# saforem2/l2hmc

Hardware: AMD Instinct MI355X
Metric: leapfrog-steps/sec (whole node), 8x8 U(1) batch 2048, 10 LF (higher is better)
Workload: dtype f32; 1 GPU; U(1) 8x8 lattice, beta=2.0, batch 2048 per GPU, 10 LF steps, GenericNet H=512 (BASELINE.json configs[2]); global_batch=2048, num_steps=10, parallelism=chains sharded over 1 GPU(s) (weak scaling), weights replicated

## Files before the change

include/l2hmc_hip.h:

```cpp
#ifndef L2HMC_HIP_H
#define L2HMC_HIP_H

#include <stddef.h>
#include <stdint.h>

#ifdef __cplusplus
extern "C" {
#endif

#define L2HMC_OK 0
#define L2HMC_ERR_ARG 1
#define L2HMC_ERR_HIP 2
#define L2HMC_ERR_WORKSPACE 3

#define L2HMC_ABI_VERSION 1

typedef void* l2hmc_stream_t;

int l2hmc_abi_version(void);
const char* l2hmc_last_error(void);

int l2hmc_u1_action_force(const float* x, int64_t rows, int32_t T, int32_t X, float beta,
                          float* action, float* force, float* avg_plaq, float* top_charge,
                          l2hmc_stream_t stream);
// ... 49 lines not shown
int l2hmc_lf_update_v(const float* v, const float* grad, const float* S, const float* T,
                      const float* Q, float eps, int32_t dir, int64_t rows, int32_t D,
                      float* v_out, float* logdet, l2hmc_stream_t stream);
int l2hmc_lf_update_x(const float* x, const float* v, const float* keep, const float* S,
                      const float* T, const float* Q, float eps, int32_t dir, int64_t rows,
                      int32_t D, float* x_out, float* logdet, l2hmc_stream_t stream);

int l2hmc_accept_prob(const float* h_old, const float* h_new, const float* sumlogdet, int64_t n,
                      float* p, l2hmc_stream_t stream);

int l2hmc_mix_accept(const float* x, const float* xf, const float* vf, const float* pf,
                     const float* xb, const float* vb, const float* pb, const float* coin,
                     const float* u, int32_t strict, int64_t B, int32_t D, float* x_prop,
                     float* v_prop, float* p, float* x_out, l2hmc_stream_t stream);

#define L2HMC_PLAN_LAYERED 1
#define L2HMC_PLAN_CONV3D 2
#define L2HMC_PLAN_SELECTED_ONLY 4
#define L2HMC_PLAN_RECOMPUTE 8
#define L2HMC_PLAN_TILES16_ONLY 16
#define L2HMC_PLAN_ALL_COLUMNS 32
#define L2HMC_PLAN_FULL_L1 64
#define L2HMC_PLAN_SINGLE_KICKS 128
typedef struct l2hmc_gauge_plan {
  int32_t T, X;
  int32_t num_steps;
  int32_t hmc;
  float eps;
  int32_t flags;
  const float* masks;
  l2hmc_dense_net xnet;
  l2hmc_dense_net vnet;
  l2hmc_conv3d_front xfront;
  l2hmc_conv3d_front vfront;
  const void* heads;
} l2hmc_gauge_plan;

size_t l2hmc_gauge_pack_heads_bytes(const l2hmc_gauge_plan* plan);
int l2hmc_gauge_pack_heads(const l2hmc_gauge_plan* plan, void* heads, l2hmc_stream_t stream);

size_t l2hmc_gauge_ws_bytes(const l2hmc_gauge_plan* plan, int64_t rows);

int l2hmc_gauge_plan_fused(const l2hmc_gauge_plan* plan);

int l2hmc_gauge_step_plan(int64_t rows_all, int32_t cus, int64_t* rows_out, int32_t* rows_per_wg_out);

// ... 207 lines not shown
```

l2hmc_amd/_lib.py:

```python
import ctypes as C
import os
import re

import torch

_HERE = os.path.dirname(os.path.abspath(__file__))
LIB_PATH = os.environ.get("L2HMC_LIB_PATH") or os.path.join(_HERE, "libl2hmc_hip.so")
HEADER_PATH = os.path.join(os.path.dirname(_HERE), "include", "l2hmc_hip.h")

c_float_p = C.c_void_p
MAX_MIX, MAX_SMALL_DIM, MAX_SMALL_NODES = 8, 8, 64
PLAN_LAYERED, PLAN_CONV3D, PLAN_SELECTED_ONLY, PLAN_RECOMPUTE, PLAN_TILES16_ONLY, PLAN_ALL_COLUMNS = 1, 2, 4, 8, 16, 32
PLAN_FULL_L1 = 64
PLAN_SINGLE_KICKS = 128
GRAD_BUCKET_REST = 6
BUCKET_FN = C.CFUNCTYPE(None, C.c_void_p, C.c_int32)


class DenseNet(C.Structure):
    _fields_ = [("D", C.c_int32), ("H", C.c_int32), ("Ka", C.c_int32), ("Kb", C.c_int32),
                ("w1_t", c_float_p), ("wt", c_float_p), ("b1", c_float_p), ("wh_t", c_float_p),
                ("bh", c_float_p), ("whd_t", c_float_p), ("bhd", c_float_p),
                ("coeff_s", c_float_p), ("coeff_q", c_float_p),
                ("q_tanh", C.c_int32), ("reserved", C.c_int32), ("packed", c_float_p)]


class DenseGrads(C.Structure):
    _fields_ = [(n, c_float_p) for n in ("w1_t", "wt", "b1", "wh_t", "bh", "whd_t", "bhd", "coeff_s", "coeff_q")]


class Conv3DGrads(C.Structure):
    _fields_ = [(n, c_float_p) for n in ("w1_a", "b1_a", "w2_a", "b2_a", "w1_b", "b1_b", "w2_b", "b2_b")]


class Conv3DFront(C.Structure):
    _fields_ = [("F", C.c_int32), ("reserved", C.c_int32),
                ("w1_a", c_float_p), ("b1_a", c_float_p), ("w2_a", c_float_p), ("b2_a", c_float_p),
# ... 228 lines not shown
```

l2hmc_amd/csrc/fused_args.h:

```cpp
#pragma once
#include "stq_dense.h"

namespace l2hmc {

struct FusedArgs {
  int T, X, num_steps, step_begin, step_end;
  float eps, beta;
  const float* masks;
  l2hmc_dense_net xnet, vnet;
  l2hmc_conv3d_front xfront, vfront;
  const float* x0; const float* v0;
  const int* dir;
  int64_t x_mod;
  int64_t dir_split;
  int64_t rows;
  float* x_out; float* v_out;
  float* logdet;
  int logdet_accumulate;
  float* p_accept;
  unsigned long long* stamps;
  int stagger;
  FusedTape tx, tv;
  float* step_x_next;
  float* step_xprop; float* step_vprop; float* step_xout;
  int64_t step_B;
  int64_t step_Bl, step_chain0;
  int step_sums_acc;
  unsigned long long step_seed, step_draw;
  int step_both;
  float* step_px; float* step_act; float* step_plq; float* step_chg; float* step_dq;
  float* step_sums;
  float* step_part;
  int step_split;
  float* step_hand;
  int* step_ticket;
  const int* heads_meta;
  const float* heads_img;
  const float* l1_img;
  int single_kicks;
};

size_t fused4_pack_floats(const l2hmc_dense_net* n);
int launch_fused4_pack(const l2hmc_dense_net* n, float* image4, hipStream_t stream);
int fused4_rows_per_wg(int64_t rows, int cus);
int launch_fused4(const FusedArgs& a, int rows_per_wg, hipStream_t stream);

int fused32_supported(const l2hmc_dense_net* n);
int launch_fused32(const FusedArgs& a, hipStream_t stream);

}
```

l2hmc_amd/csrc/fused_common.h:

```cpp
#pragma once
#include "stq_dense.h"
#include <math.h>

namespace l2hmc {

using f32x4 = __attribute__((ext_vector_type(4))) float;

constexpr int kFM = 16;
#ifndef L2HMC_FUSED_WAVES
#define L2HMC_FUSED_WAVES 4
#endif
constexpr int kFWaves = L2HMC_FUSED_WAVES;
constexpr int kFThreads = 64 * kFWaves;
constexpr int kTPC = kFThreads / kFM;


#ifdef L2HMC_TAPE_TEMPORAL
__device__ __forceinline__ void tape_store(float* dst, const f32x4& v) { *reinterpret_cast<f32x4*>(dst) = v; }
__device__ __forceinline__ f32x4 tape_load(const float* src) { return *reinterpret_cast<const f32x4*>(src); }
#else
__device__ __forceinline__ void tape_store(float* dst, const f32x4& v) {
  __builtin_nontemporal_store(v, reinterpret_cast<f32x4*>(dst));
}
__device__ __forceinline__ f32x4 tape_load(const float* src) {
// ... 32 lines not shown

template <int NT, int DEPTH, int NTI = NT, int TS = 1>
__device__ __forceinline__ void ring_prime(BRing<NT, DEPTH>& R, const float* __restrict__ wp, bool rev = false,
                                           int nkc = 0, int toff = 0) {
  const WSection ws = wsection(wp);
#pragma unroll
  for (int s = 0; s < DEPTH - 1; ++s) load_frags<NT, NTI, TS>(R.b[s], ws, rev ? nkc - 1 - s : s, toff);
  load_group<NT, 0, (NT + 1) / 2, NTI, TS>(R.b[DEPTH - 1], ws, rev ? nkc - DEPTH : DEPTH - 1, toff);
}

template <int G, int NLD, int MPL = 4, int g = 0>
__device__ __forceinline__ void sched_mfma_load_pipeline() {
  if constexpr (g < G) {
    __builtin_amdgcn_sched_group_barrier(0x008, MPL, 0);
    if constexpr (g < NLD) __builtin_amdgcn_sched_group_barrier(0x020, g == G - 1 ? NLD - g : 1, 0);
    sched_mfma_load_pipeline<G, NLD, MPL, g + 1>();
  }
}

template <int NT, int T0, int T1, int L0, int L1, bool LOAD, int NDS = 0, int NTI = NT, int TS = 1>
__device__ __forceinline__ void mfma_half_stream(const f32x4 a, const f32x4 (&cur)[NT], f32x4 (&dst)[NT],
                                                 f32x4 (&acc)[NT], const WSection& wp, int kc, int toff = 0) {
  constexpr int G = T1 - T0, NLD = L1 - L0;
#pragma unroll
  for (int i = 0; i < 4 * G; ++i) {
    const int e = i / G, t = T0 + i % G;
    acc[t] = __builtin_amdgcn_mfma_f32_16x16x4f32(cur[t][e], a[e], acc[t], 0, 0, 0);
  }
  if constexpr (LOAD) {
#pragma unroll
    for (int j = 0; j < NLD; ++j) dst[L0 + j] = lane_frag(wp, (unsigned)(kc * NTI + toff + (L0 + j) * TS));
  }
  if constexpr (NDS > 0) __builtin_amdgcn_sched_group_barrier(0x100, NDS, 0);
  sched_mfma_load_pipeline<G, LOAD ? NLD : 0>();
}

template <int NT, int NKC, int DEPTH, int NTI = NT, int TS = 1, typename AF>
__device__ __forceinline__ void stream_layer(BRing<NT, DEPTH>& R, const float* __restrict__ wbase, AF afrag,
                                             f32x4 (&acc)[NT], bool rev = false, int toff = 0) {
  const WSection wp = wsection(wbase);
  static_assert(DEPTH >= 2 && NKC >= DEPTH && NT >= 2, "ring depth / tile groups");
  constexpr int G = (NT + 1) / 2;
  auto km = [&](int k) { return rev ? NKC - 1 - k : k; };
  constexpr int MAIN = (NKC - DEPTH) / DEPTH * DEPTH;
  __builtin_amdgcn_sched_barrier(0);
  f32x4 a0 = afrag(km(0));
  int kc = 0;
#pragma nounroll
  for (; kc < MAIN; kc += DEPTH) {
#pragma unroll
    for (int s = 0; s < DEPTH; ++s) {
      const f32x4 a1 = afrag(km(kc + s + 1));
      mfma_half_stream<NT, 0, G, G, NT, true, 1, NTI, TS>(a0, R.b[s], R.b[(s + DEPTH - 1) % DEPTH], acc, wp,
                                                          km(kc + s + DEPTH - 1), toff);
      mfma_half_stream<NT, G, NT, 0, G, true, 0, NTI, TS>(a0, R.b[s], R.b[s], acc, wp, km(kc + s + DEPTH), toff);
      a0 = a1;
    }
  }
#pragma unroll
  for (int k = MAIN; k < NKC; ++k) {
    const int s = (k - MAIN) % DEPTH;
    const f32x4 a1 = afrag(km(k + 1 < NKC ? k + 1 : NKC - 1));
    if (k + DEPTH - 1 < NKC)
      mfma_half_stream<NT, 0, G, G, NT, true, 1, NTI, TS>(a0, R.b[s], R.b[(s + DEPTH - 1) % DEPTH], acc, wp,
// ... 14 lines not shown
```

l2hmc_amd/csrc/fused_traj.hip:

```cpp
#include "fused_step.h"
#include "lf_update.h"
#include <atomic>
#include <stdlib.h>

namespace l2hmc {

template <int D, int H, int KA = D, bool CONV = false>
struct FusedCfg {
  static constexpr int IMGW = CONV ? 2 * kFWaves : kFWaves;
  static constexpr int WAVES = 2 * kFWaves;
  static constexpr int RW = WAVES / IMGW;
  static constexpr int THREADS = 64 * WAVES;
  static constexpr int TPC = CONV ? THREADS / kFM : 16;
  static constexpr int SX = D + 8;
  static constexpr int SA = KA + 8;
  static constexpr int SH = H + 8;
  static constexpr int NT1 = H / (16 * WAVES);
  static constexpr int NTH = D / (16 * WAVES);
  static constexpr int NTI1 = H / (16 * IMGW);
  static constexpr int NTIH = D / (16 * IMGW);
  static_assert(NT1 >= 1 && NT1 <= 8 && NTH >= 1, "every wave needs at least one tile per layer");
  static_assert(RW == 1 || NTH == 1, "a shared heads section is walked with one tile per head and wave");
  static constexpr int KC1 = 2 * KA / 16;
  static constexpr int KC2 = H / 16;
  static constexpr size_t P1 = (size_t)2 * KA * H;
  static constexpr size_t P2 = (size_t)H * H;
  static constexpr size_t PH = (size_t)3 * D * H;
  static constexpr int NC = 4 * H + 5 * D;
  static constexpr int CF = 8, CL = 8;
  static constexpr int CW = 18 * CF + CF + 8 * CF * CF + 2 * CF;
  static constexpr int CXIN = (CL + 2) * (CL + 2) * 2;
  static constexpr int CP1 = (CL / 2 + 1) * (CL / 2 + 1) * CF;
  static constexpr int CONV_FLOATS = CONV ? 2 * kFM * SA + 4 * CW + kFM * (CXIN + CP1) : 0;
  static constexpr int ACT_FLOATS = CONV ? 0 : kFM * SX + D + 4 + D + 2 * kFM;
  static constexpr int LDS_FLOATS = 3 * kFM * SX + 2 * kFM * SH + 2 * NC + kFM * (D / 2 + 4)  +
                                    2 * D  + WAVES * kFM  + (RW > 1 ? IMGW * 64 : 0)  + kFM  +
                                    8 * kFM  + CONV_FLOATS + ACT_FLOATS;
};

__global__ void pack_fused_kernel(l2hmc_dense_net n, float* __restrict__ out, int waves) {
  const int kFWaves = waves;
  const int D = n.D, H = n.H, K1 = n.Ka + n.Kb;
  const size_t P1 = (size_t)K1 * H, P2 = (size_t)H * H, PH = (size_t)3 * D * H;
  const int NT1 = H / (16 * kFWaves), NTH = D / (16 * kFWaves);
  for (size_t i = (size_t)blockIdx.x * blockDim.x + threadIdx.x; i < P1 + P2 + PH;
       i += (size_t)gridDim.x * blockDim.x) {
    const int j = (int)(i & 3), lane = (int)((i >> 2) & 63);
    size_t rest;
    float val;
    if (i < P1 + P2) {
      const bool first = i < P1;
      const int K = first ? K1 : H;
      rest = (first ? i : i - P1) >> 8;
      const int t = (int)(rest % NT1);
      rest /= NT1;
      const int KC = K / 16;
      const int kc = (int)(rest % KC), w = (int)(rest / KC);
      const int col = (w * NT1 + t) * 16 + (lane & 15);
      const int k = kc * 16 + (lane >> 4) * 4 + j;
      val = first ? n.w1_t[(size_t)col * K1 + k] : n.wh_t[(size_t)col * H + k];
// ... 150 lines not shown
  const int sdw = wg.sdw;
  float* spx = wg.spx;
  stage_chains<kFM, kFThreads, D, SX>(p, wg, xs, vs, sdir);
  load_consts<kFThreads, D, H>(p.xnet, cx, tid);
  load_consts<kFThreads, D, H>(p.vnet, cv, tid);
  if constexpr (CONV) {
    constexpr int F = Cfg::CF, F2 = 2 * Cfg::CF;
    auto load_filters = [&](const float* w1, const float* b1, const float* w2, const float* b2, float* dst) {
      for (int i = tid; i < 18 * F; i += kFThreads) dst[i] = w1[i];
      for (int i = tid; i < F; i += kFThreads) dst[18 * F + i] = b1[i];
      for (int i = tid; i < 4 * F * F2; i += kFThreads) {
        const int g = i % F2, c = (i / F2) % F, tap = i / (F2 * F);
        dst[19 * F + i] = w2[((size_t)(tap * 2) * F + c) * F2 + g];
      }
      for (int i = tid; i < F2; i += kFThreads) dst[19 * F + 4 * F * F2 + i] = b2[i];
    };
    load_filters(p.xfront.w1_a, p.xfront.b1_a, p.xfront.w2_a, p.xfront.b2_a, cwl + 0 * Cfg::CW);
    load_filters(p.xfront.w1_b, p.xfront.b1_b, p.xfront.w2_b, p.xfront.b2_b, cwl + 1 * Cfg::CW);
    load_filters(p.vfront.w1_a, p.vfront.b1_a, p.vfront.w2_a, p.vfront.b2_a, cwl + 2 * Cfg::CW);
    load_filters(p.vfront.w1_b, p.vfront.b1_b, p.vfront.w2_b, p.vfront.b2_b, cwl + 3 * Cfg::CW);
    for (int i = tid; i < kFM * (Cfg::CXIN + Cfg::CP1); i += kFThreads) cxin[i] = 0.f;
  }
  if (tid < IMGW * kFM) ldw[tid] = 0.f;
  if constexpr (!CONV) {
    if (tid < 2 * kFM) spz[tid] = 0.f;
  }
  __syncthreads();

  const int dirl = sdir[r];

  const ChainLanes cl = chain_lanes<kFM, kTPC, 1>(p, tid);
  float act0[1], kin0[1];
  force_pass<kFM, kTPC, 1, D, SX, SP>(cl, xs, sp, gs, act0);
  kinetic_pass<kFM, kTPC, 1, D, SX>(cl, vs, kin0);

  [[maybe_unused]] auto conv_features = [&](const float* src, const float* cw, float* dst) {
    constexpr int F = Cfg::CF, F2 = 2 * Cfg::CF, L = Cfg::CL, LP = L + 2, L2 = L / 2, L2P = L2 + 1, L4 = L / 4;
    const float* w1 = cw;
    const float* b1 = cw + 18 * F;
    const float* w2 = b1 + F;
    const float* b2 = w2 + 4 * F * F2;
    for (int i = tid; i < kFM * D; i += kFThreads) {
      const int c = i / D, e = i - c * D;
      const int site = e >> 1, mu = e & 1, ii = site / L, jj = site - ii * L;
      cxin[c * Cfg::CXIN + ((ii + 1) * LP + jj + 1) * 2 + mu] = src[c * SX + e];
    }
// ... 81 lines not shown
                  }
              }
        }
        const float m0 = fmaxf(fmaxf(acc[0][0][0], acc[0][1][0]), fmaxf(acc[1][0][0], acc[1][1][0]));
        const float m1 = fmaxf(fmaxf(acc[0][0][1], acc[0][1][1]), fmaxf(acc[1][0][1], acc[1][1][1]));
        *reinterpret_cast<f32x2*>(dst + c * SA + (I2 * L4 + J2) * F2 + 2 * gp) = f32x2{fmaxf(m0, 0.f), fmaxf(m1, 0.f)};
      }
    }
    __syncthreads();
  };

  constexpr bool KEEP1 = !CONV && !TAPE && Cfg::NTH == 1 && RW == 2 && kFWaves == 8;
  f32x4 keep_v[NT1];
  [[maybe_unused]] f32x4 keep_x_own[KEEP1 ? 1 : NT1];
  f32x4 (&keep_x)[NT1] = *[&]() {
    if constexpr (KEEP1) return &keep_v;
    else return &keep_x_own;
  }();
  bool keep_v_valid = false;
  constexpr bool ACTOK = !CONV && !TAPE && Cfg::NTH == 1 && RW == 2 && kFWaves == 8;
  int arow = 0;
  constexpr bool PAIROK = !CONV && !TAPE && Cfg::NTH == 1 && RW == 2 && kFWaves == 8;

  auto net_update = [&](const l2hmc_dense_net& net, const float* cn, const float* in1, int mode, int sub,
                        bool prep_next_mask, int l1, bool is_vnet, const float tcr, const float tsr,
                        int callidx, bool pair, const float tcr2, const float tsr2) {
    const float* pk = net.packed;
    const bool zig = (callidx & 1) != 0;
    [[maybe_unused]] const FusedTape& tp = is_vnet ? p.tv : p.tx;
    [[maybe_unused]] const size_t tcr0 = (size_t)callidx * (size_t)p.rows + (size_t)row0;
    if constexpr (TAPE) {
      {
        const float* stsrc = mode == 1 ? vs : xs;
        for (int i = tid; i < kFM * (D / 4); i += kFThreads) {
          const int rr = i / (D / 4), c4 = (i - rr * (D / 4)) * 4;
          if (rr < nrow) {
            float* dst = tp.in + (tcr0 + rr) * (2 * D);
            tape_store(dst + c4, *reinterpret_cast<const f32x4*>(in1 + rr * SX + c4));
            tape_store(dst + D + c4, *reinterpret_cast<const f32x4*>(gs + rr * SX + c4));
            tape_store(tp.st + (tcr0 + rr) * D + c4, *reinterpret_cast<const f32x4*>(stsrc + rr * SX + c4));
          }
        }
      }
    }
    [[maybe_unused]] auto tape_rows = [&](float* dst, const float* src) {
      for (int i = tid; i < kFM * (H / 4); i += kFThreads) {
// ... 5 lines not shown
    const int wv = __builtin_amdgcn_readfirstlane(wave);
    const int wimg = wv / RW, wsub = wv - wimg * RW;
    const float* wp1 = pk + (size_t)wimg * Cfg::KC1 * NTI1 * 256;
    const float* wp2 = pk + Cfg::P1 + (size_t)wimg * Cfg::KC2 * NTI1 * 256;
    const float* wph = pk + Cfg::P1 + Cfg::P2 + (size_t)wimg * Cfg::KC2 * 3 * NTIH * 256;
    const int to1 = wsub * NT1, toh = wsub * NTH;
    int asense = 0;
    bool actv = false;
    const float* wpa = nullptr;
    if (ACTOK && SPLIT && mode == 2 && p.heads_img) {
      asense = sdw ^ sub;
      actv = __builtin_amdgcn_readfirstlane(sel[asense]) != 0;
      wpa = p.heads_img + ((size_t)(arow * 2 + asense) * 4 + (wv & 3)) * Cfg::KC2 * 3 * 256;
    }
    const bool l1c = ACTOK && SPLIT && p.l1_img && p.heads_img && __builtin_amdgcn_readfirstlane(sel[0] & sel[1]) != 0;
    [[maybe_unused]] float ld_k[4] = {0.f, 0.f, 0.f, 0.f}, ld_s[4] = {0.f, 0.f, 0.f, 0.f};
#ifndef L2HMC_DP1
#define L2HMC_DP1 3
#define L2HMC_DP2 3
#define L2HMC_DPH 4
#endif
    constexpr int DP1 = L2HMC_DP1, DP2 = L2HMC_DP2, DPH = L2HMC_DPH;
    BRing<NT1, DP2> R2;
    BRing<3 * NTH, DPH> R3;
#ifndef L2HMC_DP2P
#define L2HMC_DP2P 2
#define L2HMC_DPHP 3
#endif
    constexpr int DP2P = L2HMC_DP2P, DPHP = L2HMC_DPHP;
    [[maybe_unused]] BRing<NTI1, DP2P> R2P;
    [[maybe_unused]] BRing<3 * NTIH, DPHP> R3P;
    {
      constexpr int KH = Cfg::KC1 / 2;
      f32x4 acc[NT1];
      [[maybe_unused]] unsigned long long t0 = L2HMC_CYCLES_NOW();
      const float* src1 = in1;
      const float* src2 = gs;
      int s1 = SX;
      if constexpr (CONV) {
        const float* cwn = cwl + (is_vnet ? 2 : 0) * Cfg::CW;
        [[maybe_unused]] const unsigned long long tc0 = L2HMC_CYCLES_NOW();
        if (l1 == 0 || l1 == 1 || l1 == 3) conv_features(in1, cwn, fa);
        if (l1 != 2) conv_features(gs, cwn + Cfg::CW, fb);
        L2HMC_CYCLES_ADD(ft, 8, tc0);
        src1 = fa;
        src2 = fb;
        s1 = SA;
// ... 185 lines not shown
              const f32x4 mf = *reinterpret_cast<const f32x4*>(skm + c0);
              const f32x4 mb = *reinterpret_cast<const f32x4*>(skm + D + c0);
              const f32x4 x = *reinterpret_cast<const f32x4*>(xs + idx);
              f32x4 kx;
#pragma unroll
              for (int e = 0; e < 4; ++e) kx[e] = keep_of(mf[e], mb[e], d, 0) * x[e];
              if (l1n) {
#pragma unroll
                for (int e = 0; e < 4; ++e) {
                  if (keep_of(mf[e], mb[e], d, 0) != 0.f) stg[r * SX + scp[c0 + e]] = kx[e];
                  else if (kx[e] != kx[e]) spz[r] = kx[e];
                }
              } else {
                *reinterpret_cast<f32x4*>(gs + idx) = kx;
              }
            }
          }
          L2HMC_CYCLES_ADD(ft, 5, t0);
          {
            [[maybe_unused]] const unsigned long long tb = L2HMC_CYCLES_NOW();
            __syncthreads();
            L2HMC_CYCLES_ADD(ft, 6, tb);
          }
          return;
        }
      }
      ring_prime<NT1, DP2, NTI1>(R2, wp2, zig, Cfg::KC2, to1);
      L2HMC_CYCLES_ADD(ft, 0, t0);
      t0 = L2HMC_CYCLES_NOW();
      [[maybe_unused]] unsigned gmask = 0;
#pragma unroll
      for (int t = 0; t < NT1; ++t) {
        const int c0 = (wave * NT1 + t) * 16 + q * 4;
        const f32x4 b = *reinterpret_cast<const f32x4*>(cn + c0);
        const f32x4 w0 = *reinterpret_cast<const f32x4*>(cn + H + c0);
        const f32x4 w1 = *reinterpret_cast<const f32x4*>(cn + 2 * H + c0);
        f32x4 hv;
#pragma unroll
        for (int e = 0; e < 4; ++e) {
          hv[e] = fmaxf(acc[t][e] + b[e] + (tcr * w0[e] + tsr * w1[e]), 0.f);
          if constexpr (TAPE) gmask |= (hv[e] > 0.f ? 1u : 0u) << (t * 4 + e);
        }
        *reinterpret_cast<f32x4*>(h1 + r * SH + c0) = hv;
      }
      if constexpr (TAPE) {
        const size_t word = ((size_t)(callidx * 2 + 0) * gridDim.x + blockIdx.x) * (64 * IMGW) + wimg * 64 + lane;
        if constexpr (RW == 1) tp.gate[word] = gmask;
        else reinterpret_cast<unsigned short*>(tp.gate)[word * 2 + wsub] = (unsigned short)gmask;
      }
      L2HMC_CYCLES_ADD(ft, 3, t0);
    }
    {
      [[maybe_unused]] const unsigned long long tb = L2HMC_CYCLES_NOW();
      __syncthreads();
      L2HMC_CYCLES_ADD(ft, 6, tb);
    }
    if constexpr (TAPE) tape_rows(tp.h1, h1);
    {
      f32x4 acc[NT1];
#pragma unroll
      for (int t = 0; t < NT1; ++t) acc[t] = f32x4{0.f, 0.f, 0.f, 0.f};
      const float* a = h1 + r * SH + q * 4;
      [[maybe_unused]] unsigned long long t0 = L2HMC_CYCLES_NOW();
      stream_layer<NT1, Cfg::KC2, DP2, NTI1>(
          R2, wp2, [&](int kc) { return *reinterpret_cast<const f32x4*>(a + kc * 16); }, acc, zig, to1);
      if (ACTOK && actv) {
        if (wv < 4) ring_prime<3 * NTH, DPH, 3, 1>(R3, wpa, zig, Cfg::KC2, 0);
      } else {
        ring_prime<3 * NTH, DPH, 3 * NTIH, TSH>(R3, wph, zig, Cfg::KC2, toh);
      }
      L2HMC_CYCLES_ADD(ft, 1, t0);
      t0 = L2HMC_CYCLES_NOW();
      [[maybe_unused]] unsigned gmask = 0;
#pragma unroll
      for (int t = 0; t < NT1; ++t) {
        const int c0 = (wave * NT1 + t) * 16 + q * 4;
        const f32x4 b = *reinterpret_cast<const f32x4*>(cn + 3 * H + c0);
        f32x4 hv;
#pragma unroll
        for (int e = 0; e < 4; ++e) {
          hv[e] = fmaxf(acc[t][e] + b[e], 0.f);
          if constexpr (TAPE) gmask |= (hv[e] > 0.f ? 1u : 0u) << (t * 4 + e);
        }
        *reinterpret_cast<f32x4*>(h2 + r * SH + c0) = hv;
      }
      if constexpr (TAPE) {
        const size_t word = ((size_t)(callidx * 2 + 1) * gridDim.x + blockIdx.x) * (64 * IMGW) + wimg * 64 + lane;
        if constexpr (RW == 1) tp.gate[word] = gmask;
        else reinterpret_cast<unsigned short*>(tp.gate)[word * 2 + wsub] = (unsigned short)gmask;
      }
      L2HMC_CYCLES_ADD(ft, 4, t0);
    }
    {
      [[maybe_unused]] const unsigned long long tb = L2HMC_CYCLES_NOW();
      __syncthreads();
      L2HMC_CYCLES_ADD(ft, 6, tb);
    }
    if constexpr (TAPE) tape_rows(tp.h2, h2);
    {
      f32x4 acc[3 * NTH];
#pragma unroll
      for (int t = 0; t < 3 * NTH; ++t) acc[t] = f32x4{0.f, 0.f, 0.f, 0.f};
      const float* a = h2 + r * SH + q * 4;
      [[maybe_unused]] unsigned long long t0 = L2HMC_CYCLES_NOW();
      if (ACTOK && actv) {
        if (wv < 4)
          stream_layer<3 * NTH, Cfg::KC2, DPH, 3, 1>(
              R3, wpa, [&](int kc) { return *reinterpret_cast<const f32x4*>(a + kc * 16); }, acc, zig, 0);
      } else {
        stream_layer<3 * NTH, Cfg::KC2, DPH, 3 * NTIH, TSH>(
            R3, wph, [&](int kc) { return *reinterpret_cast<const f32x4*>(a + kc * 16); }, acc, zig, toh);
      }
      L2HMC_CYCLES_ADD(ft, 2, t0);
      t0 = L2HMC_CYCLES_NOW();
      float ld = 0.f;
      const float* bhd = cn + 4 * H;
      const float* es = bhd + 3 * D;
      const float* eq = es + D;
      const int d = dirl;
      if (ACTOK && actv) {
        const int* al = scol + asense * (D / 2);
        const int* il = scol + (asense ^ 1) * (D / 2);
        if (wv < 4) {
#pragma unroll
          for (int e = 0; e < 4; ++e) {
            const int c = al[wv * 16 + q * 4 + e];
            const int idx = r * SX + c;
            float S, Tt, Q, s, omk;
            heads_stq(acc[0][e], acc[1][e], acc[2][e], bhd[c], bhd[D + c], bhd[2 * D + c], es[c], eq[c], net.q_tanh, S,
                      Tt, Q);
            const float xn = lf_drift<ExpFast>(xs[idx], vs[idx], keep_of(skm[c], skm[D + c], d, sub), S, Tt, Q, eps, d, s,
                                               omk);
            xs[idx] = xn;
            stg[idx] = omk * s;
            if (prep_next_mask) gs[l1c ? r * SX + scp[c] : idx] = omk * xn;
          }
        } else {
#pragma unroll
          for (int e = 0; e < 4; ++e) {
            const int c = il[(wv - 4) * 16 + q * 4 + e];
            const int idx = r * SX + c;
            stg[idx] = 0.f;
            if (prep_next_mask) {
              const float kx = (1.f - keep_of(skm[c], skm[D + c], d, sub)) * xs[idx];
              if (!l1c) gs[idx] = kx;
              else if (kx != kx) spz[kFM + r] = kx;
            }
          }
          if (l1c && wv == 4 && q == 0) spz[sub * kFM + r] = 0.f;
        }
      } else {
#pragma unroll
      for (int t = 0; t < NTH; ++t) {
        const int c0 = wave * (D / kFWaves) + t * 16 + q * 4;
        const f32x4 b_s = *reinterpret_cast<const f32x4*>(bhd + c0);
        const f32x4 b_t = *reinterpret_cast<const f32x4*>(bhd + D + c0);
        const f32x4 b_q = *reinterpret_cast<const f32x4*>(bhd + 2 * D + c0);
        const f32x4 e_s = *reinterpret_cast<const f32x4*>(es + c0);
        const f32x4 e_q = *reinterpret_cast<const f32x4*>(eq + c0);
        const f32x4 mf = *reinterpret_cast<const f32x4*>(skm + c0);
        const f32x4 mb = *reinterpret_cast<const f32x4*>(skm + D + c0);
        const int idx = r * SX + c0;
        f32x4 S, Tt, Q;
#pragma unroll
        for (int e = 0; e < 4; ++e) {
          float s_, t_, q_;
          heads_stq(acc[0 * NTH + t][e], acc[1 * NTH + t][e], acc[2 * NTH + t][e], b_s[e], b_t[e], b_q[e], e_s[e], e_q[e],
                    net.q_tanh, s_, t_, q_);
          S[e] = s_; Tt[e] = t_; Q[e] = q_;
        }
        if constexpr (TAPE) {
          if (r < nrow) {
            const size_t plane = (size_t)p.rows * D;
// ... 62 lines not shown
      L2HMC_CYCLES_ADD(ft, 6, tb);
    }
    if (ACTOK && actv) {
      if (wsub == 1) {
        float ld = 0.f;
#pragma unroll
        for (int h = 0; h < 2; ++h)
#pragma unroll
          for (int e = 0; e < 4; ++e) ld += stg[r * SX + (2 * wimg + h) * 16 + q * 4 + e];
        ld += __shfl_xor(ld, 16, 64);
        ld += __shfl_xor(ld, 32, 64);
        if (q == 0) ldw[wimg * kFM + r] += ld;
      }
    } else if constexpr (RW > 1) {
      if (wsub == 1) {
        float ld = ldx[wimg * 64 + lane];
#pragma unroll
        for (int e = 0; e < 4; ++e) ld += ld_k[e] * ld_s[e];
        ld += __shfl_xor(ld, 16, 64);
        ld += __shfl_xor(ld, 32, 64);
        if (q == 0) ldw[wimg * kFM + r] += ld;
      }
    }
  };

  const float two_pi = 6.28318530717958647692f;
  auto step_time = [&](int step, float& tc, float& ts) {
    const int sf = step, sb = p.num_steps - 1 - step;
    const float af = two_pi * (float)sf / (float)p.num_steps, ab = two_pi * (float)sb / (float)p.num_steps;
    const float tcf = cosf(af), tsf = sinf(af), tcb = cosf(ab), tsb = sinf(ab);
    tc = dirl ? tcb : tcf;
    ts = dirl ? tsb : tsf;
  };
  auto load_step_masks = [&](int step) {
    const int sf = step, sb = p.num_steps - 1 - step;
    for (int i = tid; i < D; i += kFThreads) {
      skm[i] = p.masks[(size_t)sf * D + i];
      skm[D + i] = p.masks[(size_t)sb * D + i];
    }
    if (ACTOK && SPLIT && p.heads_meta) {
      arow = sdw ? sb : sf;
      for (int i = tid; i < D; i += kFThreads) scol[i] = p.heads_meta[2 * p.num_steps + arow * D + i];
      if (tid < 2) sel[tid] = p.heads_meta[arow * 2 + tid];
      if (p.l1_img)
        for (int i = tid; i < D; i += kFThreads) scp[i] = p.heads_meta[2 * p.num_steps + (p.num_steps + arow) * D + i];
    }
// ... 9 lines not shown
      __syncthreads();
    }
#pragma nounroll
    for (int call = paired_in ? 1 : 0; call < 4; ++call) {
      const bool is_v = call == 0 || call == 3;
      const bool pair = pair_out && call == 3;
      if (call == 3) {
        [[maybe_unused]] const unsigned long long tf = L2HMC_CYCLES_NOW();
        float unused[1];
        force_pass<kFM, kTPC, 1, D, SX, SP>(cl, xs, sp, gs, unused);
        L2HMC_CYCLES_ADD(ft, 7, tf);
        if (pair) {
          load_step_masks(step + 1);
          step_time(step + 1, tcr2, tsr2);
        }
      }
      const int l1 = call == 0 ? (keep_v_valid ? 2 : 0) : call == 1 ? 3 : call == 2 ? 4 : 1;
      net_update(is_v ? p.vnet : p.xnet, is_v ? cv : cx, is_v ? xs : vs, is_v ? 1 : 2, call == 2 ? 1 : 0,
                 call < 2, l1, is_v, tcr, tsr, 2 * step + (call == 0 || call == 1 ? 0 : 1), pair, tcr2, tsr2);
    }
    keep_v_valid = true;
    paired_in = pair_out;
  }

  float act1[1], kin1[1];
  force_pass<kFM, kTPC, 1, D, SX, SP>(cl, xs, sp, gs, act1);
  kinetic_pass<kFM, kTPC, 1, D, SX>(cl, vs, kin1);
  if (STEPM) {
    step_accept_probs<kFM, 1, IMGW>(cl, ldw, act0, act1, kin0, kin1, spx);
    __syncthreads();
    const float* xfr = xs;
    const float* xbr = xs + (kFM / 2) * SX;
    const float* vfr = vs;
    const float* vbr = vs + (kFM / 2) * SX;
    const float* pfr = spx;
    const float* pbr = spx + kFM / 2;
    if (SPLIT) {
      constexpr int HW = 2 * kFM * D + kFM;
      float* mine = p.step_hand + (size_t)blockIdx.x * HW;
      for (int i = tid; i < kFM * (D / 4); i += kFThreads) {
        const int rr = i / (D / 4), c4 = (i - rr * (D / 4)) * 4;
        *reinterpret_cast<f32x4*>(mine + rr * D + c4) = *reinterpret_cast<const f32x4*>(xs + rr * SX + c4);
        if (p.step_vprop)
          *reinterpret_cast<f32x4*>(mine + (kFM + rr) * D + c4) = *reinterpret_cast<const f32x4*>(vs + rr * SX + c4);
      }
      if (tid < kFM) mine[2 * kFM * D + tid] = spx[tid];
// ... 235 lines not shown
  L2HMC_REQUIRE(x_in && (x_next || x_out) && B > 0 && (!step_sums || part) && hand, "fused step: bad arguments");
  const int ndir = both ? 2 : 1;
  StepPart parts[3];
  const int nparts = plan_step_parts(B * ndir, !conv && subtile_enabled(p), device_cu_count(), parts);
  auto part_of = [&](int64_t c0, int64_t nb, int rpw, int accumulate) {
    const int cpw = both ? rpw / 2 : rpw;
    const int64_t D = 2 * (int64_t)p->T * p->X;
    FusedArgs a{};
    a.T = p->T; a.X = p->X; a.num_steps = p->num_steps; a.step_begin = 0; a.step_end = p->num_steps;
    a.eps = p->eps; a.beta = beta; a.masks = p->masks; a.xnet = p->xnet; a.vnet = p->vnet;
    a.xfront = p->xfront; a.vfront = p->vfront;
    a.x0 = x_in + c0 * D; a.rows = ceil_div(nb, cpw) * rpw;
    a.step_x_next = x_next ? x_next + c0 * D : nullptr;
    a.step_xprop = x_prop ? x_prop + c0 * D : nullptr;
    a.step_vprop = v_prop ? v_prop + c0 * D : nullptr;
    a.step_xout = x_out ? x_out + c0 * D : nullptr;
    a.step_B = B; a.step_Bl = nb; a.step_chain0 = c0; a.step_sums_acc = accumulate;
    a.step_seed = seed; a.step_draw = draw; a.step_both = both;
    a.step_px = px ? px + c0 : nullptr; a.step_act = actions ? actions + c0 : nullptr;
    a.step_plq = plaqs ? plaqs + c0 : nullptr; a.step_chg = charges ? charges + c0 : nullptr;
    a.step_dq = dq ? dq + c0 : nullptr;
    a.step_sums = step_sums; a.step_part = part;
    a.single_kicks = (p->flags & L2HMC_PLAN_SINGLE_KICKS) != 0;
#ifdef L2HMC_STAMPS
    a.stamps = g_stamp_cls == 5 ? g_stamp_buf : nullptr;
    a.stagger = g_fused_stagger;
#endif
    return a;
  };
  const bool split = !conv && both;
  const int* hmeta = nullptr;
  const float* himg = nullptr;
  const float* l1img = nullptr;
  if (split && p->heads && !(p->flags & L2HMC_PLAN_ALL_COLUMNS)) {
    const int Dp = 2 * p->T * p->X;
    hmeta = reinterpret_cast<const int*>(p->heads);
    himg = reinterpret_cast<const float*>(reinterpret_cast<const char*>(p->heads) + heads_meta_bytes(p->num_steps, Dp));
    if (!(p->flags & L2HMC_PLAN_FULL_L1))
      l1img = reinterpret_cast<const float*>(reinterpret_cast<const char*>(himg) +
                                             heads_sections_bytes(p->num_steps, Dp, p->xnet.H));
  }
  auto launch16 = [&](FusedArgs a) {
    if (split) {
      const int64_t pairs = ceil_div(a.step_Bl, (int64_t)kFM);
      a.rows = 2 * pairs * kFM;
      a.step_split = 1;
// ... 80 lines not shown
```

l2hmc_amd/gauge_dynamics.py:

```python
import ctypes as C

import numpy as np
import numpy.random as npr
import torch

from . import _lib, ops
from . import autograd as _autograd
from .network import ConvNet3D, GenericNet


class GaugeDynamics:

    def __init__(self, lattice, potential_fn, **kwargs):
        self.name = 'GaugeDynamics'
        self.lattice = lattice
        self.potential = potential_fn
        self.batch_size = self.lattice.samples.shape[0]
        self.x_dim = self.lattice.num_links
        self.hmc, self.network_arch, self.num_steps = False, 'generic', 5
        self.eps_trainable, self.data_format = True, 'channels_last'
        self.both_directions = True
        self.fused = True
        self.check_numerics = False
        self.recompute = False
        self.tiles16_only = False
        self.all_columns = False
        self.full_l1 = False
        self.single_kicks = False
        for key, val in kwargs.items():
            if key != 'eps':
                setattr(self, key, val)
        self._device = kwargs.get('device') or torch.device("cuda", torch.cuda.current_device())
        if getattr(potential_fn, "u1_lattice", None) is None:
            raise NotImplementedError(
                "the fused trajectory integrates the 2D U(1) action; pass lattice.get_energy_function()")
        self.eps = torch.tensor(float(kwargs.get('eps', 0.4)), dtype=torch.float32)
        self._construct_time()
        self._construct_masks_while()
        if self.hmc:
            self.position_fn = lambda inp: [torch.zeros_like(inp[0]) for _ in range(3)]
            self.momentum_fn = lambda inp: [torch.zeros_like(inp[0]) for _ in range(3)]
        elif self.network_arch == 'generic':
            self._build_generic_nets()
        elif self.network_arch == 'conv3D':
            self._build_conv_nets_3D()
        elif self.network_arch == 'conv2D':
            raise NotImplementedError(
                "network_arch='conv2D' is out of scope (SURVEY.md section 2: not named by any benchmark "
                "config, and its 4-D outputs break the reference's own reduce_sum(axis=1))")
        else:
            raise AttributeError("`self._network_arch` must be one of `'conv3D', 'conv2D', 'generic'.`")
# ... 50 lines not shown
    @property
    def variables(self):
        v = [self.eps]
        if not self.hmc:
            v += self.position_fn.variables + self.momentum_fn.variables
        return v

    @property
    def trainable_variables(self):
        v = [self.eps] if self.eps_trainable else []
        if not self.hmc:
            v += self.position_fn.trainable_variables + self.momentum_fn.trainable_variables
        return v

    def _plan(self):
        p = _lib.GaugePlan(T=self.lattice.time_size, X=self.lattice.space_size, num_steps=self.num_steps,
                           hmc=int(bool(self.hmc)), eps=float(self.eps.detach()),
                           flags=(0 if self.fused else _lib.PLAN_LAYERED)
                           | (0 if self.both_directions else _lib.PLAN_SELECTED_ONLY)
                           | (_lib.PLAN_RECOMPUTE if self.recompute else 0)
                           | (_lib.PLAN_TILES16_ONLY if self.tiles16_only else 0)
                           | (_lib.PLAN_ALL_COLUMNS if self.all_columns else 0)
                           | (_lib.PLAN_FULL_L1 if self.full_l1 else 0)
                           | (_lib.PLAN_SINGLE_KICKS if self.single_kicks else 0),
                           masks=_lib.dev_ptr(self.mask, name="mask"))
        if not self.hmc:
            p.xnet = self.position_fn.pack()
            p.vnet = self.momentum_fn.pack()
            if self.network_arch == 'conv3D':
                p.flags |= _lib.PLAN_CONV3D
                p.xfront = self.position_fn.pack_front()
                p.vfront = self.momentum_fn.pack_front()
            elif self.fused:
                p.heads = self._heads_image(p)
        return p

    def _heads_image(self, plan):
        L = _lib.lib()
        nbytes = L.l2hmc_gauge_pack_heads_bytes(C.byref(plan))
        if not nbytes:
            return None
        key = (plan.xnet.whd_t, getattr(self.position_fn, "_pack_serial", 0))
        h = getattr(self, "_heads", None)
        if h is None or h[0] is not self.mask or h[1] != key or h[2].numel() * 4 < nbytes:
            buf = torch.empty(nbytes // 4, dtype=torch.float32, device=self._device)
            _lib.call("l2hmc_gauge_pack_heads", C.byref(plan), buf, device=self._device)
            self._heads = h = (self.mask, key, buf)
# ... 144 lines not shown
```

Before: 16.18 million chain-leapfrog-steps/s.

## Split fused head GEMM across all eight waves with LDS exchange

In the fused trajectory kernel's active-column head path, the three head output tiles were computed by waves 0-3 alone while waves 4-7 only handled the kept columns. Now waves 0-3 stream two head tiles and waves 4-7 stream the third. Partial results are swapped through LDS behind an added barrier, and every wave finishes two moved and two kept columns. This spreads head MFMA and weight streaming over twice the waves, at the cost of an extra __syncthreads and LDS traffic. The old single-wave-group behaviour is kept behind a new HEADS_ONE_WAVE plan flag, and optional per-phase stamp accumulation in LDS is added for profiling builds.

Measured after the change: 16.28 million chain-leapfrog-steps/s (median of 6 runs). No clear change (+0.6%).

```diff
diff --git a/include/l2hmc_hip.h b/include/l2hmc_hip.h
--- a/include/l2hmc_hip.h
+++ b/include/l2hmc_hip.h
@@ -95,6 +95,7 @@
 #define L2HMC_PLAN_ALL_COLUMNS 32
 #define L2HMC_PLAN_FULL_L1 64
 #define L2HMC_PLAN_SINGLE_KICKS 128
+#define L2HMC_PLAN_HEADS_ONE_WAVE 256
 typedef struct l2hmc_gauge_plan {
   int32_t T, X;
   int32_t num_steps;
diff --git a/l2hmc_amd/_lib.py b/l2hmc_amd/_lib.py
--- a/l2hmc_amd/_lib.py
+++ b/l2hmc_amd/_lib.py
@@ -13,6 +13,7 @@
 PLAN_LAYERED, PLAN_CONV3D, PLAN_SELECTED_ONLY, PLAN_RECOMPUTE, PLAN_TILES16_ONLY, PLAN_ALL_COLUMNS = 1, 2, 4, 8, 16, 32
 PLAN_FULL_L1 = 64
 PLAN_SINGLE_KICKS = 128
+PLAN_HEADS_ONE_WAVE = 256
 GRAD_BUCKET_REST = 6
 BUCKET_FN = C.CFUNCTYPE(None, C.c_void_p, C.c_int32)
 
diff --git a/l2hmc_amd/csrc/fused_args.h b/l2hmc_amd/csrc/fused_args.h
--- a/l2hmc_amd/csrc/fused_args.h
+++ b/l2hmc_amd/csrc/fused_args.h
@@ -38,6 +38,7 @@
   const float* heads_img;
   const float* l1_img;
   int single_kicks;
+  int heads_one_wave;
 };
 
 size_t fused4_pack_floats(const l2hmc_dense_net* n);
diff --git a/l2hmc_amd/csrc/fused_common.h b/l2hmc_amd/csrc/fused_common.h
--- a/l2hmc_amd/csrc/fused_common.h
+++ b/l2hmc_amd/csrc/fused_common.h
@@ -78,9 +78,10 @@
 __device__ __forceinline__ void mfma_half_stream(const f32x4 a, const f32x4 (&cur)[NT], f32x4 (&dst)[NT],
                                                  f32x4 (&acc)[NT], const WSection& wp, int kc, int toff = 0) {
   constexpr int G = T1 - T0, NLD = L1 - L0;
+  constexpr int GD = G > 0 ? G : 1;
 #pragma unroll
   for (int i = 0; i < 4 * G; ++i) {
-    const int e = i / G, t = T0 + i % G;
+    const int e = i / GD, t = T0 + i % GD;
     acc[t] = __builtin_amdgcn_mfma_f32_16x16x4f32(cur[t][e], a[e], acc[t], 0, 0, 0);
   }
   if constexpr (LOAD) {
@@ -89,13 +90,14 @@
   }
   if constexpr (NDS > 0) __builtin_amdgcn_sched_group_barrier(0x100, NDS, 0);
   sched_mfma_load_pipeline<G, LOAD ? NLD : 0>();
+  if constexpr (G == 0 && LOAD && NLD > 0) __builtin_amdgcn_sched_group_barrier(0x020, NLD, 0);
 }
 
 template <int NT, int NKC, int DEPTH, int NTI = NT, int TS = 1, typename AF>
 __device__ __forceinline__ void stream_layer(BRing<NT, DEPTH>& R, const float* __restrict__ wbase, AF afrag,
                                              f32x4 (&acc)[NT], bool rev = false, int toff = 0) {
   const WSection wp = wsection(wbase);
-  static_assert(DEPTH >= 2 && NKC >= DEPTH && NT >= 2, "ring depth / tile groups");
+  static_assert(DEPTH >= 2 && NKC >= DEPTH && NT >= 1, "ring depth / tile groups");
   constexpr int G = (NT + 1) / 2;
   auto km = [&](int k) { return rev ? NKC - 1 - k : k; };
   constexpr int MAIN = (NKC - DEPTH) / DEPTH * DEPTH;
diff --git a/l2hmc_amd/csrc/fused_traj.hip b/l2hmc_amd/csrc/fused_traj.hip
--- a/l2hmc_amd/csrc/fused_traj.hip
+++ b/l2hmc_amd/csrc/fused_traj.hip
@@ -33,9 +33,14 @@
   static constexpr int CP1 = (CL / 2 + 1) * (CL / 2 + 1) * CF;
   static constexpr int CONV_FLOATS = CONV ? 2 * kFM * SA + 4 * CW + kFM * (CXIN + CP1) : 0;
   static constexpr int ACT_FLOATS = CONV ? 0 : kFM * SX + D + 4 + D + 2 * kFM;
+#ifdef L2HMC_STAMPS
+  static constexpr int STAMP_FLOATS = 128;
+#else
+  static constexpr int STAMP_FLOATS = 0;
+#endif
   static constexpr int LDS_FLOATS = 3 * kFM * SX + 2 * kFM * SH + 2 * NC + kFM * (D / 2 + 4)  +
                                     2 * D  + WAVES * kFM  + (RW > 1 ? IMGW * 64 : 0)  + kFM  +
-                                    8 * kFM  + CONV_FLOATS + ACT_FLOATS;
+                                    8 * kFM  + CONV_FLOATS + ACT_FLOATS + STAMP_FLOATS;
 };
 
 __global__ void pack_fused_kernel(l2hmc_dense_net n, float* __restrict__ out, int waves) {
@@ -232,6 +237,11 @@
     for (int i = tid; i < kFM * (Cfg::CXIN + Cfg::CP1); i += kFThreads) cxin[i] = 0.f;
   }
   if (tid < IMGW * kFM) ldw[tid] = 0.f;
+#ifdef L2HMC_STAMPS
+  static_assert((Cfg::LDS_FLOATS - Cfg::STAMP_FLOATS) % 2 == 0, "the stamp sums are 64-bit");
+  unsigned long long* sst = reinterpret_cast<unsigned long long*>(lds + (Cfg::LDS_FLOATS - Cfg::STAMP_FLOATS));
+  if (tid < Cfg::STAMP_FLOATS / 2) sst[tid] = 0ull;
+#endif
   if constexpr (!CONV) {
     if (tid < 2 * kFM) spz[tid] = 0.f;
   }
@@ -359,6 +369,17 @@
   int arow = 0;
   constexpr bool PAIROK = !CONV && !TAPE && Cfg::NTH == 1 && RW == 2 && kFWaves == 8;
 
+  [[maybe_unused]] auto flush_stamps = [&](int kind) {
+#ifdef L2HMC_STAMPS
+    if (p.step_B > 0) {
+      if (lane == 0 && (wave == 0 || wave == 4)) {
+        unsigned long long* dst = sst + ((wave >> 2) * 3 + kind) * 10;
+        for (int i = 0; i < 9; ++i) dst[i] += ft[i];
+      }
+      for (int i = 0; i < 9; ++i) ft[i] = 0;
+    }
+#endif
+  };
   auto net_update = [&](const l2hmc_dense_net& net, const float* cn, const float* in1, int mode, int sub,
                         bool prep_next_mask, int l1, bool is_vnet, const float tcr, const float tsr,
                         int callidx, bool pair, const float tcr2, const float tsr2) {
@@ -410,7 +431,15 @@
 #endif
     constexpr int DP1 = L2HMC_DP1, DP2 = L2HMC_DP2, DPH = L2HMC_DPH;
     BRing<NT1, DP2> R2;
-    BRing<3 * NTH, DPH> R3;
+    union {
+      BRing<3 * NTH, DPH> R3;
+      BRing<2, DPH> R3E;
+      BRing<1, DPH> R3O;
+    } RH;
+    BRing<3 * NTH, DPH>& R3 = RH.R3;
+    [[maybe_unused]] BRing<2, DPH>& R3E = RH.R3E;
+    [[maybe_unused]] BRing<1, DPH>& R3O = RH.R3O;
+    const bool two = ACTOK && actv && !p.heads_one_wave;
 #ifndef L2HMC_DP2P
 #define L2HMC_DP2P 2
 #define L2HMC_DPHP 3
@@ -642,6 +671,7 @@
             __syncthreads();
             L2HMC_CYCLES_ADD(ft, 6, tb);
           }
+          flush_stamps(0);
           return;
         }
       }
@@ -684,7 +714,10 @@
       [[maybe_unused]] unsigned long long t0 = L2HMC_CYCLES_NOW();
       stream_layer<NT1, Cfg::KC2, DP2, NTI1>(
           R2, wp2, [&](int kc) { return *reinterpret_cast<const f32x4*>(a + kc * 16); }, acc, zig, to1);
-      if (ACTOK && actv) {
+      if (ACTOK && two) {
+        if (wv < 4) ring_prime<2, DPH, 3, 1>(R3E, wpa, zig, Cfg::KC2, 0);
+        else ring_prime<1, DPH, 3, 1>(R3O, wpa, zig, Cfg::KC2, 2);
+      } else if (ACTOK && actv) {
         if (wv < 4) ring_prime<3 * NTH, DPH, 3, 1>(R3, wpa, zig, Cfg::KC2, 0);
       } else {
         ring_prime<3 * NTH, DPH, 3 * NTIH, TSH>(R3, wph, zig, Cfg::KC2, toh);
@@ -723,7 +756,21 @@
       for (int t = 0; t < 3 * NTH; ++t) acc[t] = f32x4{0.f, 0.f, 0.f, 0.f};
       const float* a = h2 + r * SH + q * 4;
       [[maybe_unused]] unsigned long long t0 = L2HMC_CYCLES_NOW();
-      if (ACTOK && actv) {
+      float* hx = h1;
+      if (ACTOK && two) {
+        if (wv < 4) {
+          f32x4 acc2[2] = {f32x4{0.f, 0.f, 0.f, 0.f}, f32x4{0.f, 0.f, 0.f, 0.f}};
+          stream_layer<2, Cfg::KC2, DPH, 3, 1>(
+              R3E, wpa, [&](int kc) { return *reinterpret_cast<const f32x4*>(a + kc * 16); }, acc2, zig, 0);
+          acc[0] = acc2[0];
+          acc[1] = acc2[1];
+        } else {
+          f32x4 acc1[1] = {f32x4{0.f, 0.f, 0.f, 0.f}};
+          stream_layer<1, Cfg::KC2, DPH, 3, 1>(
+              R3O, wpa, [&](int kc) { return *reinterpret_cast<const f32x4*>(a + kc * 16); }, acc1, zig, 2);
+          acc[2] = acc1[0];
+        }
+      } else if (ACTOK && actv) {
         if (wv < 4)
           stream_layer<3 * NTH, Cfg::KC2, DPH, 3, 1>(
               R3, wpa, [&](int kc) { return *reinterpret_cast<const f32x4*>(a + kc * 16); }, acc, zig, 0);
@@ -741,34 +788,85 @@
       if (ACTOK && actv) {
         const int* al = scol + asense * (D / 2);
         const int* il = scol + (asense ^ 1) * (D / 2);
-        if (wv < 4) {
-#pragma unroll
-          for (int e = 0; e < 4; ++e) {
-            const int c = al[wv * 16 + q * 4 + e];
-            const int idx = r * SX + c;
-            float S, Tt, Q, s, omk;
-            heads_stq(acc[0][e], acc[1][e], acc[2][e], bhd[c], bhd[D + c], bhd[2 * D + c], es[c], eq[c], net.q_tanh, S,
-                      Tt, Q);
-            const float xn = lf_drift<ExpFast>(xs[idx], vs[idx], keep_of(skm[c], skm[D + c], d, sub), S, Tt, Q, eps, d, s,
-                                               omk);
-            xs[idx] = xn;
-            stg[idx] = omk * s;
-            if (prep_next_mask) gs[l1c ? r * SX + scp[c] : idx] = omk * xn;
+        struct Moved { int idx, gidx; float xn, ls, kx; };
+        auto move_column = [&](int sec, int e, float aS, float aT, float aQ) {
+          const int c = al[sec * 16 + q * 4 + e];
+          const int idx = r * SX + c;
+          float S, Tt, Q, s, omk;
+          heads_stq(aS, aT, aQ, bhd[c], bhd[D + c], bhd[2 * D + c], es[c], eq[c], net.q_tanh, S, Tt, Q);
+          const float xn = lf_drift<ExpFast>(xs[idx], vs[idx], keep_of(skm[c], skm[D + c], d, sub), S, Tt, Q, eps, d, s,
+                                             omk);
+          Moved m;
+          m.idx = idx;
+          m.xn = xn;
+          m.ls = omk * s;
+          m.gidx = prep_next_mask && l1c ? r * SX + scp[c] : idx;
+          m.kx = omk * xn;
+          return m;
+        };
+        auto put_moved = [&](const Moved& m) {
+          xs[m.idx] = m.xn;
+          stg[m.idx] = m.ls;
+          if (prep_next_mask) gs[m.gidx] = m.kx;
+        };
+        struct Kept { int idx; float kx; };
+        auto keep_column = [&](int sec, int e) {
+          const int c = il[sec * 16 + q * 4 + e];
+          Kept k;
+          k.idx = r * SX + c;
+          k.kx = 0.f;
+          if (prep_next_mask) k.kx = (1.f - keep_of(skm[c], skm[D + c], d, sub)) * xs[k.idx];
+          return k;
+        };
+        auto put_kept = [&](const Kept& k) {
+          stg[k.idx] = 0.f;
+          if (prep_next_mask) {
+            if (!l1c) gs[k.idx] = k.kx;
+            else if (k.kx != k.kx) spz[kFM + r] = k.kx;
+          }
+        };
+        if (!two) {
+          if (wv < 4) {
+#pragma unroll
+            for (int e = 0; e < 4; ++e) put_moved(move_column(wv, e, acc[0][e], acc[1][e], acc[2][e]));
+          } else {
+#pragma unroll
+            for (int e = 0; e < 4; ++e) put_kept(keep_column(wv - 4, e));
           }
         } else {
-#pragma unroll
-          for (int e = 0; e < 4; ++e) {
-            const int c = il[(wv - 4) * 16 + q * 4 + e];
-            const int idx = r * SX + c;
-            stg[idx] = 0.f;
-            if (prep_next_mask) {
-              const float kx = (1.f - keep_of(skm[c], skm[D + c], d, sub)) * xs[idx];
-              if (!l1c) gs[idx] = kx;
-              else if (kx != kx) spz[kFM + r] = kx;
-            }
-          }
-          if (l1c && wv == 4 && q == 0) spz[sub * kFM + r] = 0.f;
-        }
+          using f32x2 = __attribute__((ext_vector_type(2))) float;
+          f32x2* hxs = reinterpret_cast<f32x2*>(hx) + (wv & 3) * 3 * 64 + lane;
+          if (wv < 4) {
+            hxs[0] = f32x2{acc[0][2], acc[0][3]};
+            hxs[64] = f32x2{acc[1][2], acc[1][3]};
+          } else {
+            hxs[128] = f32x2{acc[2][0], acc[2][1]};
+          }
+          L2HMC_CYCLES_ADD(ft, 5, t0);
+          {
+            [[maybe_unused]] const unsigned long long tb = L2HMC_CYCLES_NOW();
+            __syncthreads();
+            L2HMC_CYCLES_ADD(ft, 6, tb);
+          }
+          t0 = L2HMC_CYCLES_NOW();
+          const int sec = wv & 3, e0 = wv < 4 ? 0 : 2;
+          float a_s[2], a_t[2], a_q[2];
+          if (wv < 4) {
+            const f32x2 aq = hxs[128];
+            a_s[0] = acc[0][0]; a_s[1] = acc[0][1]; a_t[0] = acc[1][0]; a_t[1] = acc[1][1]; a_q[0] = aq[0]; a_q[1] = aq[1];
+          } else {
+            const f32x2 as = hxs[0], at = hxs[64];
+            a_s[0] = as[0]; a_s[1] = as[1]; a_t[0] = at[0]; a_t[1] = at[1]; a_q[0] = acc[2][2]; a_q[1] = acc[2][3];
+          }
+          const Moved m0 = move_column(sec, e0, a_s[0], a_t[0], a_q[0]);
+          const Moved m1 = move_column(sec, e0 + 1, a_s[1], a_t[1], a_q[1]);
+          const Kept k0 = keep_column(sec, e0), k1 = keep_column(sec, e0 + 1);
+          put_moved(m0);
+          put_moved(m1);
+          put_kept(k0);
+          put_kept(k1);
+        }
+        if (l1c && wv == 4 && q == 0) spz[sub * kFM + r] = 0.f;
       } else {
 #pragma unroll
       for (int t = 0; t < NTH; ++t) {
@@ -877,6 +975,7 @@
         if (q == 0) ldw[wimg * kFM + r] += ld;
       }
     }
+    flush_stamps(mode == 1 ? 0 : 1 + sub);
   };
 
   const float two_pi = 6.28318530717958647692f;
@@ -932,6 +1031,19 @@
     keep_v_valid = true;
     paired_in = pair_out;
   }
+#ifdef L2HMC_STAMPS
+  if (p.step_B > 0 && p.stamps) {
+    __syncthreads();
+    if (tid == 0) {
+      unsigned long long rt1;
+      asm volatile("s_memrealtime %0\n\ts_waitcnt lgkmcnt(0)" : "=s"(rt1)::"memory");
+      for (int i = 0; i < 60; ++i) p.stamps[blockIdx.x * 64 + i] = sst[i];
+      p.stamps[blockIdx.x * 64 + 60] = L2HMC_CYCLES_NOW() - ft_start;
+      p.stamps[blockIdx.x * 64 + 61] = rt0;
+      p.stamps[blockIdx.x * 64 + 62] = rt1;
+    }
+  }
+#endif
 
   float act1[1], kin1[1];
   force_pass<kFM, kTPC, 1, D, SX, SP>(cl, xs, sp, gs, act1);
@@ -1213,6 +1325,7 @@
     a.step_dq = dq ? dq + c0 : nullptr;
     a.step_sums = step_sums; a.step_part = part;
     a.single_kicks = (p->flags & L2HMC_PLAN_SINGLE_KICKS) != 0;
+    a.heads_one_wave = (p->flags & L2HMC_PLAN_HEADS_ONE_WAVE) != 0;
 #ifdef L2HMC_STAMPS
     a.stamps = g_stamp_cls == 5 ? g_stamp_buf : nullptr;
     a.stagger = g_fused_stagger;
diff --git a/l2hmc_amd/gauge_dynamics.py b/l2hmc_amd/gauge_dynamics.py
--- a/l2hmc_amd/gauge_dynamics.py
+++ b/l2hmc_amd/gauge_dynamics.py
@@ -27,6 +27,7 @@
         self.all_columns = False
         self.full_l1 = False
         self.single_kicks = False
+        self.heads_one_wave = False
         for key, val in kwargs.items():
             if key != 'eps':
                 setattr(self, key, val)
@@ -123,7 +124,8 @@
                            | (_lib.PLAN_TILES16_ONLY if self.tiles16_only else 0)
                            | (_lib.PLAN_ALL_COLUMNS if self.all_columns else 0)
                            | (_lib.PLAN_FULL_L1 if self.full_l1 else 0)
-                           | (_lib.PLAN_SINGLE_KICKS if self.single_kicks else 0),
+                           | (_lib.PLAN_SINGLE_KICKS if self.single_kicks else 0)
+                           | (_lib.PLAN_HEADS_ONE_WAVE if self.heads_one_wave else 0),
                            masks=_lib.dev_ptr(self.mask, name="mask"))
         if not self.hmc:
             p.xnet = self.position_fn.pack()
```
